# aluo7/ViT-SOM

Measured on AMD Instinct MI355X. Metric: images/sec/node ViT-SOM 40x40 CIFAR-10 bs512 (training step: fwd+bwd+all-reduce+AdamW), higher is better.
Workload: dtype f32 (Linear GEMMs on bf16 MFMA: forward from an exact 3xbf16 operand split, six products; weight / input gradients from a 2xbf16 split, three products, rel. error 4e-6)

## Files before the change

### include/vitsom_hip.h

```cpp
#ifndef VITSOM_HIP_H
#define VITSOM_HIP_H

#include <stddef.h>
#include <stdint.h>

#ifdef __cplusplus
extern "C" {
#endif

typedef struct ihipStream_t* vsom_stream_t;

#define VSOM_OK 0
#define VSOM_EINVAL (-1)
#define VSOM_EALIGN (-2)
#define VSOM_EUNSUPPORTED (-3)
#define VSOM_EWORKSPACE (-4)

#define VSOM_VERSION 100

#define VSOM_DIST_COSINE 0
#define VSOM_DIST_EUCLIDEAN 1
#define VSOM_DIST_MANHATTAN 2

int vsom_version(void);
// ... 39 lines not shown
                         float* dcls_token, int B, int C, int S, int p, int E, void* ws,
                         size_t ws_bytes, vsom_stream_t stream);

int vsom_layernorm_fwd(const float* X, const float* gamma, const float* beta, float* Y, float* mean,
                       float* rstd, int rows, int cols, float eps, vsom_stream_t stream);
size_t vsom_layernorm_bwd_workspace_bytes(int rows, int cols);
int vsom_layernorm_bwd(const float* dY, const float* X, const float* mean, const float* rstd,
                       const float* gamma, const float* resid, float* dX, float* dgamma, float* dbeta,
                       int rows, int cols, void* ws, size_t ws_bytes, vsom_stream_t stream);
#define VSOM_LN_JOB_WORDS 4
int vsom_layernorm_bwd_deferrable(int rows, int cols);
int vsom_layernorm_bwd_partial(const float* dY, const float* X, const float* mean, const float* rstd,
                               const float* gamma, const float* resid, float* dX, int rows, int cols, void* part,
                               size_t part_bytes, vsom_stream_t stream);
int vsom_layernorm_bwd_finish_many(const int64_t* jobs_dev, int first, int count, int max_cols, vsom_stream_t stream);

int vsom_attention_fwd(const float* qkv, float* out, float* lse, int B, int N, int H, int hd,
                       vsom_stream_t stream);
int vsom_attention_bwd(const float* qkv, const float* out, const float* dout, const float* lse,
                       float* dqkv, float* delta_ws, int B, int N, int H, int hd,
                       vsom_stream_t stream);
int vsom_attention_probs(const float* qkv, const float* lse, float* probs, int B, int N, int H, int hd,
                         vsom_stream_t stream);
int vsom_set_attention_fused(int fused);

int vsom_attention_q1_fwd(const float* q, const float* kv, float* o, float* lse, int B, int N, int H, int hd,
                          vsom_stream_t stream);
int vsom_attention_q1_bwd(const float* dout, const float* o, const float* lse, const float* q, const float* kv, float* dq,
                          float* dkv, int B, int N, int H, int hd, vsom_stream_t stream);
int vsom_rows_add(const float* src, long lds, float* dst, long ldd, int rows, int cols, vsom_stream_t stream);
// ... 122 lines not shown
```

### vit_som_amd/_lib.py

```python
import ctypes as C
import os

import torch

_HERE = os.path.dirname(os.path.abspath(__file__))
LIB_PATH = os.path.join(_HERE, "libvitsom_hip.so")

c_fp = C.c_void_p
c_stream = C.c_void_p

SIGNATURES = {
    "vsom_version": (C.c_int, []),
    "vsom_last_error_string": (C.c_char_p, []),
    "vsom_linear_fwd": (C.c_int, [c_fp, C.c_long, c_fp, c_fp, c_fp, C.c_long, C.c_int, C.c_int, C.c_int, c_stream]),
    "vsom_linear_gelu_fwd": (C.c_int, [c_fp, C.c_long, c_fp, c_fp, c_fp, c_fp, C.c_int, C.c_int, C.c_int, c_stream]),
    "vsom_linear_relu_fwd": (C.c_int, [c_fp, C.c_long, c_fp, c_fp, c_fp, c_fp, C.c_int, C.c_int, C.c_int, c_stream]),
    "vsom_l1_loss_workspace_bytes": (C.c_size_t, [C.c_long]),
    "vsom_l1_loss": (C.c_int, [c_fp, c_fp, c_fp, c_fp, C.c_float, C.c_long, c_fp, C.c_size_t, c_stream]),
    "vsom_linear_residual_fwd": (C.c_int, [c_fp, C.c_long, c_fp, c_fp, c_fp, C.c_long, C.c_int, c_fp, C.c_long,
                                           C.c_int, C.c_int, C.c_int, c_stream]),
    "vsom_linear_bwd_input": (C.c_int, [c_fp, C.c_long, c_fp, c_fp, C.c_long, C.c_int, C.c_int, C.c_int, C.c_int,
                                        c_fp, c_stream]),
    "vsom_linear_bwd_input_t": (C.c_int, [c_fp, C.c_long, c_fp, c_fp, C.c_long, C.c_int, C.c_int, C.c_int, C.c_int,
                                          c_fp, c_stream]),
# ... 2 lines not shown
    "vsom_get_gemm_mode": (C.c_int, []),
    "vsom_linear_bwd_weight_workspace_bytes": (C.c_size_t, [C.c_int, C.c_int, C.c_int]),
    "vsom_linear_bwd_weight": (C.c_int, [c_fp, C.c_long, c_fp, C.c_long, c_fp, c_fp, C.c_int, C.c_int, C.c_int,
                                         c_fp, C.c_size_t, c_stream]),
    "vsom_patch_embed_fwd": (C.c_int, [c_fp, c_fp, c_fp, c_fp, c_fp, c_fp, c_fp, C.c_int, C.c_int, C.c_int, C.c_int,
                                       C.c_int, c_stream]),
    "vsom_patch_embed_bwd_workspace_bytes": (C.c_size_t, [C.c_int] * 5),
    "vsom_patch_embed_bwd": (C.c_int, [c_fp, c_fp, c_fp, c_fp, c_fp, C.c_int, C.c_int, C.c_int, C.c_int, C.c_int,
                                       c_fp, C.c_size_t, c_stream]),
    "vsom_layernorm_fwd": (C.c_int, [c_fp, c_fp, c_fp, c_fp, c_fp, c_fp, C.c_int, C.c_int, C.c_float, c_stream]),
    "vsom_layernorm_bwd_workspace_bytes": (C.c_size_t, [C.c_int, C.c_int]),
    "vsom_layernorm_bwd": (C.c_int, [c_fp] * 9 + [C.c_int, C.c_int, c_fp, C.c_size_t, c_stream]),
    "vsom_layernorm_bwd_deferrable": (C.c_int, [C.c_int, C.c_int]),
    "vsom_layernorm_bwd_partial": (C.c_int, [c_fp] * 7 + [C.c_int, C.c_int, c_fp, C.c_size_t, c_stream]),
    "vsom_layernorm_bwd_finish_many": (C.c_int, [c_fp, C.c_int, C.c_int, C.c_int, c_stream]),
    "vsom_attention_fwd": (C.c_int, [c_fp, c_fp, c_fp, C.c_int, C.c_int, C.c_int, C.c_int, c_stream]),
    "vsom_attention_bwd": (C.c_int, [c_fp] * 6 + [C.c_int] * 4 + [c_stream]),
    "vsom_set_attention_fused": (C.c_int, [C.c_int]),
    "vsom_attention_probs": (C.c_int, [c_fp, c_fp, c_fp, C.c_int, C.c_int, C.c_int, C.c_int, c_stream]),
    "vsom_attention_q1_fwd": (C.c_int, [c_fp] * 4 + [C.c_int] * 4 + [c_stream]),
    "vsom_attention_q1_bwd": (C.c_int, [c_fp] * 7 + [C.c_int] * 4 + [c_stream]),
    "vsom_rows_add": (C.c_int, [c_fp, C.c_long, c_fp, C.c_long, C.c_int, C.c_int, c_stream]),
    "vsom_tape_begin": (C.c_int, []),
    "vsom_tape_cut": (C.c_int, []),
    "vsom_tape_pause": (C.c_int, [C.c_int]),
    "vsom_tape_end": (C.c_int, []),
    "vsom_tape_recording": (C.c_int, []),
    "vsom_tape_segment_ops": (C.c_int, [C.c_int, C.c_int]),
    "vsom_tape_replay": (C.c_int, [C.c_int, C.c_int]),
    "vsom_tape_destroy": (C.c_int, [C.c_int]),
# ... 170 lines not shown
```

### vit_som_amd/csrc/gemm_f32.h

```cpp
#pragma once
#include "common.h"

namespace vsom {

enum Epi : int {
    EPI_NONE = 0,
    EPI_BIAS = 1,
    EPI_BIAS_GELU = 2,
    EPI_BIAS_RES = 3,
    EPI_ROWAXPY = 4,
    EPI_GELU_BWD = 5,
    EPI_SLAB = 6,
    EPI_BIAS_RELU = 7,
};

struct GemmP {
    const float* A; const float* B; float* C;
    long lda, ldb, ldc;
    int M, N, K;
    int ktiles_per_split;
    int a_seg, a_stride, a_off;
    int c_seg, c_stride, c_off;
    const float* bias;
    const float* R; long ldr; int r_mod, r_off;
    float* C2; long ldc2;
    const float* rowscale;
    float alpha; int accumulate;
    float* slab; long slab_stride;
    float* slab_bias; long slab_bias_stride;
    int n_major;
    int a_vec, b_vec;
    unsigned a_bytes, b_bytes;
    int products;
};

template <int R_>
struct StageRegs { f32x4 v[R_ / 32]; };

constexpr unsigned OOB = 0xFFFFFFF0u;

__device__ __forceinline__ f32x4 bload4(__amdgpu_buffer_rsrc_t rsrc, unsigned off) {
    return __builtin_bit_cast(f32x4, __builtin_amdgcn_raw_buffer_load_b128(rsrc, (int)off, 0, 0));
}

__device__ __forceinline__ f32x4 bload4s(__amdgpu_buffer_rsrc_t rsrc, unsigned voff, unsigned soff) {
    return __builtin_bit_cast(f32x4, __builtin_amdgcn_raw_buffer_load_b128(rsrc, (int)voff, (int)soff, 0));
}

// ... 445 lines not shown
```

### vit_som_amd/csrc/gemm_f32.hip

```cpp
#include "gemm_f32.h"
#include "gemm_x6.h"
#include "gemm_x6_tn.h"

#include <atomic>

#include <stdarg.h>
#include <stdlib.h>

namespace vsom {

static thread_local char g_err[512] = "no error";
void set_error(const char* fmt, ...) {
    va_list ap;
    va_start(ap, fmt);
    vsnprintf(g_err, sizeof(g_err), fmt, ap);
    va_end(ap);
}
const char* last_error() { return g_err; }

static std::atomic<int> g_gemm_mode{VSOM_GEMM_SPLIT_BF16_GRAD3};
int gemm_mode() { return g_gemm_mode.load(std::memory_order_relaxed); }
static bool split_engine() { return gemm_mode() != VSOM_GEMM_F32; }
int gemm_grad_products() { return gemm_mode() == VSOM_GEMM_SPLIT_BF16_GRAD3 ? 3 : 6; }

// ... 165 lines not shown
    p.cfg = (N % 192 == 0 && K % 64 == 0) ? 1 : (N % 96 == 0 && K % 96 == 0) ? 2 : 0;
    if (p.cfg == 0) {
        p.splits = choose_splits(cdiv(N, gemm_tile_m(false, false, N)) * cdiv(K, 64), cdiv(M, 32), 128);
        return p;
    }
    const int tiles = p.cfg == 1 ? (N / 192) * (K / 64) : (N / 96) * (K / 96);
    const int ktiles = cdiv(M, 32);
    int s = (384 + tiles / 2) / tiles;
    if (s > ktiles) s = ktiles;
    if (s < 1) s = 1;
    const int per = cdiv(ktiles, s);
    p.splits = cdiv(ktiles, per);
    return p;
}
static long pad4(long n) { return (n + 3) & ~3L; }


int linear_bwd_weight_impl(const float* dY, long lddy, const float* X, long ldx, float* dW, float* db, int M, int N,
                           int K, int a_seg, int a_stride, int a_off, void* ws, size_t ws_bytes,
                           hipStream_t stream) {
    VSOM_REQUIRE(dY && X && dW, VSOM_EINVAL, "linear_bwd_weight: null pointer");
    VSOM_REQUIRE(lddy >= N && ldx >= K, VSOM_EINVAL, "linear_bwd_weight: leading dimension too small");
    VSOM_REQUIRE(ws && ws_bytes >= vsom_linear_bwd_weight_workspace_bytes(M, N, K), VSOM_EWORKSPACE,
                 "linear_bwd_weight: workspace too small (%zu < %zu)", ws_bytes,
                 vsom_linear_bwd_weight_workspace_bytes(M, N, K));
    VSOM_REQUIRE(aligned16(ws), VSOM_EALIGN, "linear_bwd_weight: workspace must be 16-byte aligned");
    const TnPlan plan = bwd_weight_plan(M, N, K);
    const int splits = plan.splits;
    const long wlen = pad4((long)N * K), blen = pad4(N);
    float* slab = static_cast<float*>(ws);
// ... 108 lines not shown
int vsom_linear_bwd_input_t(const float* dY, long lddy, const float* Wt, float* dX, long lddx, int M, int N, int K,
                            int accumulate, const float* gelu_grad, vsom_stream_t stream) {
    VSOM_REQUIRE(dY && Wt && dX, VSOM_EINVAL, "linear_bwd_input_t: null pointer");
    VSOM_REQUIRE(lddy >= N && lddx >= K, VSOM_EINVAL, "linear_bwd_input_t: leading dimension too small");
    GemmP g = {};
    g.A = dY; g.lda = lddy; g.B = Wt; g.ldb = N; g.C = dX; g.ldc = lddx;
    g.M = M; g.N = K; g.K = N; g.alpha = 1.f; g.accumulate = accumulate;
    g.products = gemm_grad_products();
    if (gelu_grad) {
        g.R = gelu_grad; g.ldr = K;
        return launch_gemm(true, true, EPI_GELU_BWD, g, 1, stream);
    }
    return launch_gemm(true, true, EPI_NONE, g, 1, stream);
}

int vsom_set_gemm_mode(int mode) {
    VSOM_REQUIRE(mode == VSOM_GEMM_F32 || mode == VSOM_GEMM_SPLIT_BF16 || mode == VSOM_GEMM_SPLIT_BF16_GRAD3, VSOM_EINVAL,
                 "set_gemm_mode: unknown mode %d", mode);
    g_gemm_mode.store(mode, std::memory_order_relaxed);
    return VSOM_OK;
}
int vsom_get_gemm_mode(void) { return gemm_mode(); }

size_t vsom_linear_bwd_weight_workspace_bytes(int M, int N, int K) {
    if (M <= 0 || N <= 0 || K <= 0) return 0;
    const int s = bwd_weight_plan(M, N, K).splits;
    return (size_t)s * (size_t)(pad4((long)N * K) + pad4(N)) * sizeof(float);
}

int vsom_linear_bwd_weight(const float* dY, long lddy, const float* X, long ldx, float* dW, float* db, int M,
// ... 6 lines not shown
```

### vit_som_amd/csrc/gemm_x6.h

```cpp
#pragma once
#include "gemm_f32.h"

namespace vsom {

typedef __attribute__((ext_vector_type(8))) __bf16 bf16x8;

__device__ __forceinline__ unsigned x6_bits(float x) { return __builtin_bit_cast(unsigned, x); }
__device__ __forceinline__ float x6_float(unsigned x) { return __builtin_bit_cast(float, x); }

__device__ __forceinline__ void x6_split(f32x4 v, uint2& p1, uint2& p2, uint2& p3) {
    const unsigned HI = 0xffff0000u, SEL = 0x07060302u;
    float r[4], s[4];
#pragma unroll
    for (int e = 0; e < 4; ++e) {
        r[e] = v[e] - x6_float(x6_bits(v[e]) & HI);
        s[e] = r[e] - x6_float(x6_bits(r[e]) & HI);
    }
    p1.x = __builtin_amdgcn_perm(x6_bits(v[1]), x6_bits(v[0]), SEL); p1.y = __builtin_amdgcn_perm(x6_bits(v[3]), x6_bits(v[2]), SEL);
    p2.x = __builtin_amdgcn_perm(x6_bits(r[1]), x6_bits(r[0]), SEL); p2.y = __builtin_amdgcn_perm(x6_bits(r[3]), x6_bits(r[2]), SEL);
    p3.x = __builtin_amdgcn_perm(x6_bits(s[1]), x6_bits(s[0]), SEL); p3.y = __builtin_amdgcn_perm(x6_bits(s[3]), x6_bits(s[2]), SEL);
}

typedef __attribute__((ext_vector_type(2))) __bf16 bf16x2_t;
__device__ __forceinline__ void x3_split(f32x4 v, uint2& p1, uint2& p2) {
// ... 36 lines not shown
}
template <int NPL = 3>
__device__ __forceinline__ void x6_store_ks(const X6Blk& b, char* planes, int plane_bytes, int mq, int kg) {
#pragma unroll
    for (int e = 0; e < 4; ++e) {
        const f32x4 col = {b.v[0][e], b.v[1][e], b.v[2][e], b.v[3][e]};
        uint2 p1, p2, p3;
        if constexpr (NPL == 3) x6_split(col, p1, p2, p3); else x3_split(col, p1, p2);
        char* dst = planes + x6_piece_off(4 * mq + e, kg);
        *reinterpret_cast<uint2*>(dst) = p1;
        *reinterpret_cast<uint2*>(dst + plane_bytes) = p2;
        if constexpr (NPL == 3) *reinterpret_cast<uint2*>(dst + 2 * plane_bytes) = p3;
    }
}

template <bool A_KC, bool B_KC, int WM, int WN, int WAVES_M, int WAVES_N, int EPI, int NPL = 3>
__global__ __launch_bounds__(256) void gemm_x6_kernel(const GemmP g) {
    constexpr int BM = WAVES_M * WM * 32;
    constexpr int BN = WAVES_N * WN * 32;
    constexpr int PA = BM * X6_RS, PB = BN * X6_RS;
    __shared__ __attribute__((aligned(16))) char lds[NPL * (PA + PB)];
    char* As = lds;
    char* Bs = lds + NPL * PA;

    const int t = threadIdx.x;
    const int lane = t & 63, wave = t >> 6;
    const int r = lane & 31, h = lane >> 5;
    const int wm0 = (wave / WAVES_N) * (WM * 32);
    const int wn0 = (wave % WAVES_N) * (WN * 32);

    const int tiles_n = (g.N + BN - 1) / BN;
    const int tiles_m = (g.M + BM - 1) / BM;
// ... 13 lines not shown

    f32x16 acc[WM][WN];
#pragma unroll
    for (int i = 0; i < WM; ++i)
#pragma unroll
        for (int j = 0; j < WN; ++j)
#pragma unroll
            for (int v = 0; v < 16; ++v) acc[i][j][v] = 0.f;

    const __amdgpu_buffer_rsrc_t rsA = __builtin_amdgcn_make_buffer_rsrc(const_cast<float*>(g.A), 0, (int)g.a_bytes, 0x00020000);
    const __amdgpu_buffer_rsrc_t rsB = __builtin_amdgcn_make_buffer_rsrc(const_cast<float*>(g.B), 0, (int)g.b_bytes, 0x00020000);
    StageRegs<A_KC ? BM : 32> sa;
    StageRegs<B_KC ? BN : 32> sb;
    OffKC<A_KC ? BM : 32> oa; OffKC<B_KC ? BN : 32> ob;
    constexpr int TA = 2 * BM, TB0 = 256 - 2 * BN;
    static_assert(TA <= 256 && TB0 >= 0, "tile too large for the k-strided task map");
    const bool has_a = !A_KC && t < TA, has_b = !B_KC && t >= TB0;
    const int kga = t & 7, mqa = t >> 3, kgb = (t - TB0) & 7, mqb = (t - TB0) >> 3;
    X6Blk ba, bb;
    unsigned cola = OOB, colb = OOB;
    float cs[4] = {0.f, 0.f, 0.f, 0.f};
    const bool want_colsum = (EPI == EPI_SLAB) && !A_KC && g.slab_bias != nullptr && bn0 == 0;
    if constexpr (A_KC) init_kc<BM>(oa, g.lda, bm0, g.M, t);
    else if (has_a && bm0 + 4 * mqa < g.M) cola = (unsigned)(bm0 + 4 * mqa) << 2;
    if constexpr (B_KC) init_kc<BN>(ob, g.ldb, bn0, g.N, t);
    else if (has_b && bn0 + 4 * mqb < g.N) colb = (unsigned)(bn0 + 4 * mqb) << 2;
    auto gload = [&](int kt) {
        if constexpr (A_KC) load_kc_fast<BM>(sa, rsA, oa, kt << 5, g.K, t);
        else if (has_a) x6_load_ks(ba, rsA, cola, (unsigned)g.lda << 2, kt << 5, g.K, kga, g.a_seg, g.a_stride, g.a_off);
        if constexpr (B_KC) load_kc_fast<BN>(sb, rsB, ob, kt << 5, g.K, t);
        else if (has_b) x6_load_ks(bb, rsB, colb, (unsigned)g.ldb << 2, kt << 5, g.K, kgb, 0, 0, 0);
// ... 58 lines not shown
        lstore();
        __syncthreads();
    }
    if (kt_begin < kt_end) mfma_tile();
    if constexpr (EPI == EPI_SLAB && !A_KC) {
        if (want_colsum && has_a) {
#pragma unroll
            for (int e = 0; e < 4; ++e) {
                float v = cs[e];
                v += __shfl_xor(v, 1, 64); v += __shfl_xor(v, 2, 64); v += __shfl_xor(v, 4, 64);
                const int m = bm0 + 4 * mqa + e;
                if (kga == 0 && m < g.M) g.slab_bias[(long)z * g.slab_bias_stride + m] = v;
            }
        }
    }
    gemm_epilogue<WM, WN, EPI>(g, acc, bm0 + wm0, bn0 + wn0, r, h, z);
}

}
```

### vit_som_amd/csrc/layernorm.hip

```cpp
#include "gemm_f32.h"

namespace vsom {

template <int MAXV>
__global__ __launch_bounds__(256) void layernorm_fwd_kernel(const float* __restrict__ X,
                                                            const float* __restrict__ gamma,
                                                            const float* __restrict__ beta,
                                                            float* __restrict__ Y, float* __restrict__ mean,
                                                            float* __restrict__ rstd, int rows, int cols,
                                                            float eps) {
    const int lane = threadIdx.x & 63;
    const int row = blockIdx.x * 4 + (threadIdx.x >> 6);
    if (row >= rows) return;
    const float* x = X + (long)row * cols;
    float v[MAXV];
    float s = 0.f;
#pragma unroll
    for (int j = 0; j < MAXV; ++j) {
        const int c = lane + 64 * j;
        v[j] = (c < cols) ? x[c] : 0.f;
        s += v[j];
    }
    const float mu = wave_sum(s) / (float)cols;
    float q = 0.f;
// ... 64 lines not shown
            }
        }
    }
#pragma unroll
    for (int j = 0; j < MAXV; ++j) {
        const int c = lane + 64 * j;
        if (c < cols) { sh[(wave * 2 + 0) * cols + c] = dg[j]; sh[(wave * 2 + 1) * cols + c] = db[j]; }
    }
    __syncthreads();
    for (int c = threadIdx.x; c < 2 * cols; c += 256) {
        const float s = (sh[c] + sh[2 * cols + c]) + (sh[4 * cols + c] + sh[6 * cols + c]);
        part[(long)blockIdx.x * 2 * cols + c] = s;
    }
}

__device__ __forceinline__ float group16_sum(float v) {
    v += __shfl_xor(v, 8, 64); v += __shfl_xor(v, 4, 64); v += __shfl_xor(v, 2, 64); v += __shfl_xor(v, 1, 64);
    return v;
}

template <int NCH>
__global__ __launch_bounds__(256) void layernorm_fwd_v4_kernel(const float* __restrict__ X, const float* __restrict__ gamma,
                                                               const float* __restrict__ beta, float* __restrict__ Y,
                                                               float* __restrict__ mean, float* __restrict__ rstd, int rows,
                                                               int cols, float eps) {
    const int sub = threadIdx.x & 15;
    const int row = blockIdx.x * 16 + (threadIdx.x >> 4);
    const bool ok = row < rows;
    const f32x4* x = reinterpret_cast<const f32x4*>(X + (long)(ok ? row : 0) * cols);
    const float inv_n = 1.0f / (float)cols;
    f32x4 v[NCH];
    bool cv[NCH];
    float s = 0.f;
#pragma unroll
// ... 35 lines not shown
    const float inv_n = 1.0f / (float)cols;
    f32x4 gam[NCH], dg[NCH], db[NCH];
    bool cv[NCH];
#pragma unroll
    for (int j = 0; j < NCH; ++j) {
        cv[j] = 4 * (sub + 16 * j) < cols;
        gam[j] = cv[j] ? reinterpret_cast<const f32x4*>(gamma)[sub + 16 * j] : f32x4{0.f, 0.f, 0.f, 0.f};
        dg[j] = f32x4{0.f, 0.f, 0.f, 0.f};
        db[j] = f32x4{0.f, 0.f, 0.f, 0.f};
    }
    for (int row0 = blockIdx.x * 16; row0 < rows; row0 += gridDim.x * 16) {
        const int row = row0 + rg;
        const bool ok = row < rows;
        const long base = (long)(ok ? row : 0) * cols;
        const float mu = mean[ok ? row : 0], rs = rstd[ok ? row : 0];
        f32x4 xh[NCH], g[NCH];
        float s1 = 0.f, s2 = 0.f;
#pragma unroll
        for (int j = 0; j < NCH; ++j) {
            f32x4 d = f32x4{0.f, 0.f, 0.f, 0.f}, xv = f32x4{mu, mu, mu, mu};
            if (cv[j]) {
                xv = reinterpret_cast<const f32x4*>(X + base)[sub + 16 * j];
                if (ok) d = reinterpret_cast<const f32x4*>(dY + base)[sub + 16 * j];
            }
#pragma unroll
            for (int e = 0; e < 4; ++e) {
                xh[j][e] = (xv[e] - mu) * rs;
                g[j][e] = d[e] * gam[j][e];
                s1 += g[j][e];
                s2 = fmaf(g[j][e], xh[j][e], s2);
                dg[j][e] = fmaf(d[e], xh[j][e], dg[j][e]);
                db[j][e] += d[e];
            }
        }
        s1 = group16_sum(s1) * inv_n;
        s2 = group16_sum(s2) * inv_n;
        if (ok) {
#pragma unroll
            for (int j = 0; j < NCH; ++j) {
                if (!cv[j]) continue;
                f32x4 o;
#pragma unroll
                for (int e = 0; e < 4; ++e) o[e] = rs * (g[j][e] - s1 - xh[j][e] * s2);
                if (resid) {
                    const f32x4 rr = reinterpret_cast<const f32x4*>(resid + base)[sub + 16 * j];
#pragma unroll
                    for (int e = 0; e < 4; ++e) o[e] += rr[e];
                }
                reinterpret_cast<f32x4*>(dX + base)[sub + 16 * j] = o;
            }
        }
    }
#pragma unroll
    for (int j = 0; j < NCH; ++j) {
        if (!cv[j]) continue;
        reinterpret_cast<f32x4*>(sh + (rg * 2 + 0) * cols)[sub + 16 * j] = dg[j];
        reinterpret_cast<f32x4*>(sh + (rg * 2 + 1) * cols)[sub + 16 * j] = db[j];
    }
    __syncthreads();
    for (int c = threadIdx.x; c < 2 * cols; c += 256) {
        float s = 0.f;
#pragma unroll
        for (int q = 0; q < 16; ++q) s += sh[q * 2 * cols + c];
        part[(long)blockIdx.x * 2 * cols + c] = s;
// ... 114 lines not shown
```

### vit_som_amd/ops.py

```python
from typing import Optional

import torch

from . import _lib as _lib_mod
from ._lib import check, lib, ptr, stream

_scratch = {}
_retired = []

_timers = {}


def enable_timer(name: str):
    _timers[name] = []


def disable_timers():
    _timers.clear()


def timer_ms(name: str):
    ev = _timers.get(name, [])
    if not ev:
        return None
# ... 196 lines not shown
            del self.keys[i:], self.rows_host[i:], self.parts[i:]
            self.table = None
        if i == len(self.keys):
            nbytes = lib.vsom_layernorm_bwd_workspace_bytes(rows, cols)
            part = torch.empty(nbytes, dtype=torch.uint8, device=self.device)
            self.keys.append(key); self.parts.append(part)
            self.rows_host.append([ptr(part), ptr(dgamma), ptr(dbeta), ((nbytes // (8 * cols)) << 32) | cols])
            self.max_cols = max(self.max_cols, cols)
            self.table = None
        part = self.parts[i]
        check(lib.vsom_layernorm_bwd_partial(ptr(dy), ptr(x), ptr(mean), ptr(rstd), ptr(gamma), ptr(resid), ptr(dx), rows, cols,
                                             ptr(part), part.numel(), stream()), "vsom_layernorm_bwd_partial")
        self.n += 1
        return dx

    def flush(self):
        if self.n == self.flushed:
            return
        if self.table is None or self.table.shape[0] < self.n:
            self.table = torch.tensor(self.rows_host, dtype=torch.int64, device=self.device)
        check(lib.vsom_layernorm_bwd_finish_many(ptr(self.table), self.flushed, self.n - self.flushed, self.max_cols, stream()),
              "vsom_layernorm_bwd_finish_many")
        self.flushed = self.n


def layernorm_bwd_deferrable(rows: int, cols: int) -> bool:
    return bool(lib.vsom_layernorm_bwd_deferrable(int(rows), int(cols)))


def attention_fwd(qkv, out, lse, B, N, H, hd):
    assert qkv.is_contiguous() and out.is_contiguous() and lse.is_contiguous()
    _f32(qkv, "qkv")
    check(lib.vsom_attention_fwd(ptr(qkv), ptr(out), ptr(lse), B, N, H, hd, stream()), "vsom_attention_fwd")
    return out


def attention_bwd(qkv, out, dout, lse, dqkv, delta, B, N, H, hd):
    assert all(t.is_contiguous() for t in (qkv, out, dout, lse, dqkv, delta))
    check(lib.vsom_attention_bwd(ptr(qkv), ptr(out), ptr(dout), ptr(lse), ptr(dqkv), ptr(delta), B, N, H, hd, stream()),
          "vsom_attention_bwd")
    return dqkv

# ... 431 lines not shown
```

### vit_som_amd/tuning.py

```python


class _Hooks:
    side_stream = True
    fwd_split = True
    fwd_split_blocks = None
    overlap_allreduce = True
    bucket_blocks = 3
    bmu_planes = True
    adamw_planes = False
    ln_reduce_batched = True
    bmu_overlap = False
    launch_tape = True
    cls_prune = True

    def set(self, **kw):
        for k, v in kw.items():
            if not hasattr(_Hooks, k):
                raise AttributeError(f"unknown hook {k!r}")
            setattr(self, k, v)
        return self

    def signature(self):
        return tuple((k, getattr(self, k)) for k in sorted(vars(_Hooks)) if not k.startswith("_") and not callable(getattr(_Hooks, k)))

    def reset(self):
        for k in list(self.__dict__):
            delattr(self, k)
        return self
# ... 4 lines not shown
```

### vit_som_amd/vit.py

```python
import math
from typing import Dict

import numpy as np
import torch
import torch.nn as nn

from . import ops
from ._base import _Acts
from ._lib import Event, on_stream
from .tuning import hooks


def _sincos_1d(embed_dim: int, pos: np.ndarray) -> np.ndarray:
    omega = np.arange(embed_dim // 2, dtype=np.float64) / (embed_dim / 2.0)
    omega = 1.0 / 10000 ** omega
    out = np.einsum("m,d->md", pos.reshape(-1).astype(np.float64), omega)
    return np.concatenate([np.sin(out), np.cos(out)], axis=1)


def get_2d_sincos_pos_embed(embed_dim: int, grid_size: int, cls_token: bool = False) -> np.ndarray:
    gh = np.arange(grid_size, dtype=np.float32)
    gw = np.arange(grid_size, dtype=np.float32)
    grid = np.stack(np.meshgrid(gw, gh), axis=0).reshape(2, 1, grid_size, grid_size)
    emb = np.concatenate([_sincos_1d(embed_dim // 2, grid[0]), _sincos_1d(embed_dim // 2, grid[1])], axis=1)
# ... 321 lines not shown
            pend.clear()
            return
        while len(pend) > keep:
            pend.pop(0).wait()

    def _side_mark(self):
        if self._side is not None:
            self.__dict__.setdefault("_side_pending", []).append(self._event().record(self._side))

    def _ln_bwd(self, dy, x, mean, rstd, gamma, resid, dx, dgamma, dbeta):
        jobs = self.__dict__.get("_ln_jobs")
        if jobs is not None and ops.layernorm_bwd_deferrable(*x.shape):
            return jobs.bwd(dy, x, mean, rstd, gamma, resid, dx, dgamma, dbeta)
        return ops.layernorm_bwd(dy, x, mean, rstd, gamma, resid, dx, dgamma, dbeta)

    def _block_bwd(self, blk: Block, L: _Acts, x_in, gout, a: _Acts, G, prefix: str, bufs, WT=None, parity: int = 0):
        T, dim, hid = a.T, blk.dim, blk.hidden
        self._side_join(keep=1)
        g1, g0 = bufs
        dh = a.dh2[parity][:T * hid].view(T, hid)
        da = a.da[:T * dim].view(T, dim)
        dqkv = a.dqkv2[parity][:T * 3 * dim].view(T, 3 * dim)
        self._dw(gout, L.hact, G(f"{prefix}.mlp.2.weight"), G(f"{prefix}.mlp.2.bias"))
        self._dx(WT, gout, blk.mlp["2"].weight, dh, gelu_grad=L.hpre)
        self._dw(dh, L.a2, G(f"{prefix}.mlp.0.weight"), G(f"{prefix}.mlp.0.bias"))
        self._dx(WT, dh, blk.mlp["0"].weight, da)
        self._ln_bwd(da, L.x1, L.mean2, L.rstd2, blk.norm2.weight, gout, g1, G(f"{prefix}.norm2.weight"),
                          G(f"{prefix}.norm2.bias"))
        self._dw(g1, L.ao, G(f"{prefix}.attn.proj.weight"), G(f"{prefix}.attn.proj.bias"))
        self._dx(WT, g1, blk.attn.proj.weight, da)
        ops.attention_bwd(L.qkv, L.ao, da, L.lse, dqkv, a.delta, a.B, a.N, blk.heads, dim // blk.heads)
        self._dw(dqkv, L.a1, G(f"{prefix}.attn.qkv.weight"), G(f"{prefix}.attn.qkv.bias"))
        self._dx(WT, dqkv, blk.attn.qkv.weight, da)
        self._ln_bwd(da, x_in, L.mean1, L.rstd1, blk.norm1.weight, g1, g0, G(f"{prefix}.norm1.weight"),
                          G(f"{prefix}.norm1.bias"))
        self._side_mark()
        return g0

    def _views(self, a: _Acts, dim: int):
        return [b[:a.T * dim].view(a.T, dim) for b in a.g]

    def _decoder_bwd(self, a: _Acts, G, WT=None, before_dxe=None):
        DE = self.decoder_embed_dim
        ring = self._views(a, DE)
        gA = ring[0]
        ops.linear_bwd_weight(a.dpred, a.dn, G("decoder_pred.weight"), G("decoder_pred.bias"))
        dn_grad = a.da[:a.T * DE].view(a.T, DE)
        self._dx(WT, a.dpred, self.decoder_pred.weight, dn_grad)
        x_last = a.dec[-1].x2 if a.dec else a.dec0
        self._ln_bwd(dn_grad, x_last, a.mean_d, a.rstd_d, self.decoder_norm.weight, None, gA,
# ... 116 lines not shown
```

Measured before the change: 54180.

## Fuse LayerNorm backward into the input-gradient GEMM epilogue

Adds a GEMM kernel variant whose epilogue computes the LayerNorm backward for full-width row tiles (K=192 or 96). It writes dX with the residual added and emits per-tile dgamma/dbeta partials, which are reduced later or deferred through the existing LN job queue. The transformer block backward now uses this fused path for norm2 and norm1. This removes the intermediate da write/read and one kernel launch per LayerNorm. In exchange, whole-row tiles may reduce GEMM parallelism and raise register pressure.

```diff
diff --git a/include/vitsom_hip.h b/include/vitsom_hip.h
--- a/include/vitsom_hip.h
+++ b/include/vitsom_hip.h
@@ -77,6 +77,15 @@
                                const float* gamma, const float* resid, float* dX, int rows, int cols, void* part,
                                size_t part_bytes, vsom_stream_t stream);
 int vsom_layernorm_bwd_finish_many(const int64_t* jobs_dev, int first, int count, int max_cols, vsom_stream_t stream);
+
+int vsom_linear_bwd_input_ln_supported(int M, int N, int K);
+size_t vsom_linear_bwd_input_ln_partial_bytes(int M, int K);
+int vsom_linear_bwd_input_ln(const float* dY, long lddy, const float* Wt, int M, int N, int K, const float* X,
+                             const float* mean, const float* rstd, const float* gamma, const float* resid, float* dX,
+                             float* dgamma, float* dbeta, void* ws, size_t ws_bytes, vsom_stream_t stream);
+int vsom_linear_bwd_input_ln_partial(const float* dY, long lddy, const float* Wt, int M, int N, int K, const float* X,
+                                     const float* mean, const float* rstd, const float* gamma, const float* resid,
+                                     float* dX, void* part, size_t part_bytes, vsom_stream_t stream);
 
 int vsom_attention_fwd(const float* qkv, float* out, float* lse, int B, int N, int H, int hd,
                        vsom_stream_t stream);
diff --git a/vit_som_amd/_lib.py b/vit_som_amd/_lib.py
--- a/vit_som_amd/_lib.py
+++ b/vit_som_amd/_lib.py
@@ -40,6 +40,10 @@
     "vsom_layernorm_bwd_deferrable": (C.c_int, [C.c_int, C.c_int]),
     "vsom_layernorm_bwd_partial": (C.c_int, [c_fp] * 7 + [C.c_int, C.c_int, c_fp, C.c_size_t, c_stream]),
     "vsom_layernorm_bwd_finish_many": (C.c_int, [c_fp, C.c_int, C.c_int, C.c_int, c_stream]),
+    "vsom_linear_bwd_input_ln_supported": (C.c_int, [C.c_int, C.c_int, C.c_int]),
+    "vsom_linear_bwd_input_ln_partial_bytes": (C.c_size_t, [C.c_int, C.c_int]),
+    "vsom_linear_bwd_input_ln": (C.c_int, [c_fp, C.c_long, c_fp, C.c_int, C.c_int, C.c_int] + [c_fp] * 8 + [c_fp, C.c_size_t, c_stream]),
+    "vsom_linear_bwd_input_ln_partial": (C.c_int, [c_fp, C.c_long, c_fp, C.c_int, C.c_int, C.c_int] + [c_fp] * 6 + [c_fp, C.c_size_t, c_stream]),
     "vsom_attention_fwd": (C.c_int, [c_fp, c_fp, c_fp, C.c_int, C.c_int, C.c_int, C.c_int, c_stream]),
     "vsom_attention_bwd": (C.c_int, [c_fp] * 6 + [C.c_int] * 4 + [c_stream]),
     "vsom_set_attention_fused": (C.c_int, [C.c_int]),
diff --git a/vit_som_amd/csrc/gemm_f32.h b/vit_som_amd/csrc/gemm_f32.h
--- a/vit_som_amd/csrc/gemm_f32.h
+++ b/vit_som_amd/csrc/gemm_f32.h
@@ -12,6 +12,7 @@
     EPI_GELU_BWD = 5,
     EPI_SLAB = 6,
     EPI_BIAS_RELU = 7,
+    EPI_LN_BWD = 8,
 };
 
 struct GemmP {
@@ -32,6 +33,8 @@
     int a_vec, b_vec;
     unsigned a_bytes, b_bytes;
     int products;
+    const float* ln_x; const float* ln_mean; const float* ln_rstd; const float* ln_gamma; const float* ln_resid;
+    float* ln_part;
 };
 
 template <int R_>
diff --git a/vit_som_amd/csrc/gemm_f32.hip b/vit_som_amd/csrc/gemm_f32.hip
--- a/vit_som_amd/csrc/gemm_f32.hip
+++ b/vit_som_amd/csrc/gemm_f32.hip
@@ -203,6 +203,43 @@
     return p;
 }
 static long pad4(long n) { return (n + 3) & ~3L; }
+
+static bool ln_fused_width(int K) { return K == 192 || K == 96; }
+static int ln_fused_tiles(int M, int K) { return cdiv(M, K == 192 ? 64 : 128); }
+
+static int linear_bwd_input_ln_launch(const float* dY, long lddy, const float* Wt, int M, int N, int K, const float* X,
+                                      const float* mean, const float* rstd, const float* gamma, const float* resid,
+                                      float* dX, float* part, size_t part_bytes, hipStream_t stream) {
+    VSOM_REQUIRE(dY && Wt && X && mean && rstd && gamma && dX, VSOM_EINVAL, "linear_bwd_input_ln: null pointer");
+    VSOM_REQUIRE(M > 0 && N > 0 && lddy >= N, VSOM_EINVAL, "linear_bwd_input_ln: bad shape M=%d N=%d lddy=%ld", M, N, lddy);
+    VSOM_REQUIRE(vsom_linear_bwd_input_ln_supported(M, N, K), VSOM_EUNSUPPORTED,
+                 "linear_bwd_input_ln: unsupported (M=%d N=%d K=%d, gemm mode %d)", M, N, K, gemm_mode());
+    VSOM_REQUIRE(aligned16(dY) && aligned16(Wt) && aligned16(X) && aligned16(gamma) && aligned16(dX) &&
+                 (!resid || aligned16(resid)) && lddy % 4 == 0 && N % 4 == 0, VSOM_EALIGN,
+                 "linear_bwd_input_ln: operands must be 16-byte aligned (lddy, N multiples of 4)");
+    VSOM_REQUIRE(part && aligned16(part) && part_bytes >= vsom_linear_bwd_input_ln_partial_bytes(M, K), VSOM_EWORKSPACE,
+                 "linear_bwd_input_ln: partial buffer too small or misaligned");
+    const long ab = operand_bytes(M, lddy, N), bb = operand_bytes(K, N, N);
+    VSOM_REQUIRE(ab < 0xFFFF0000L && (long)M * K * 4 < 0xFFFF0000L, VSOM_EUNSUPPORTED, "linear_bwd_input_ln: operand larger than 4 GB");
+    GemmP g = {};
+    g.A = dY; g.lda = lddy; g.B = Wt; g.ldb = N; g.C = dX; g.ldc = K;
+    g.M = M; g.N = K; g.K = N; g.alpha = 1.f;
+    g.ktiles_per_split = cdiv(N, 32);
+    g.a_vec = g.b_vec = 1;
+    g.a_bytes = (unsigned)ab; g.b_bytes = (unsigned)bb;
+    g.products = gemm_grad_products();
+    g.ln_x = X; g.ln_mean = mean; g.ln_rstd = rstd; g.ln_gamma = gamma; g.ln_resid = resid; g.ln_part = part;
+    const dim3 grid(ln_fused_tiles(M, K)), block(256);
+    const bool x3 = g.products == 3;
+    if (K == 192) {
+        if (x3) VSOM_LAUNCH((gemm_x6_ln_kernel<3, 2, 2, 2>), grid, block, 0, stream, g);
+        else VSOM_LAUNCH((gemm_x6_ln_kernel<3, 2, 2, 3>), grid, block, 0, stream, g);
+    } else {
+        if (x3) VSOM_LAUNCH((gemm_x6_ln_kernel<3, 4, 1, 2>), grid, block, 0, stream, g);
+        else VSOM_LAUNCH((gemm_x6_ln_kernel<3, 4, 1, 3>), grid, block, 0, stream, g);
+    }
+    VSOM_LAUNCH_CHECK("gemm_x6_ln_kernel");
+}
 
 
 int linear_bwd_weight_impl(const float* dY, long lddy, const float* X, long ldx, float* dW, float* db, int M, int N,
@@ -341,6 +378,32 @@
     return launch_gemm(true, true, EPI_NONE, g, 1, stream);
 }
 
+int vsom_linear_bwd_input_ln_supported(int M, int N, int K) {
+    return M > 0 && N > 0 && split_engine() && ln_fused_width(K) && ln_fused_tiles(M, K) >= 32;
+}
+
+size_t vsom_linear_bwd_input_ln_partial_bytes(int M, int K) {
+    if (M <= 0 || !ln_fused_width(K)) return 0;
+    return (size_t)ln_fused_tiles(M, K) * 2 * (size_t)K * sizeof(float);
+}
+
+int vsom_linear_bwd_input_ln(const float* dY, long lddy, const float* Wt, int M, int N, int K, const float* X,
+                             const float* mean, const float* rstd, const float* gamma, const float* resid, float* dX,
+                             float* dgamma, float* dbeta, void* ws, size_t ws_bytes, vsom_stream_t stream) {
+    VSOM_REQUIRE(dgamma && dbeta, VSOM_EINVAL, "linear_bwd_input_ln: null pointer");
+    float* part = static_cast<float*>(ws);
+    const int rc = linear_bwd_input_ln_launch(dY, lddy, Wt, M, N, K, X, mean, rstd, gamma, resid, dX, part, ws_bytes, stream);
+    if (rc) return rc;
+    return reduce_slabs2_internal(part, 2L * K, ln_fused_tiles(M, K), dgamma, K, dbeta, K, K, stream);
+}
+
+int vsom_linear_bwd_input_ln_partial(const float* dY, long lddy, const float* Wt, int M, int N, int K, const float* X,
+                                     const float* mean, const float* rstd, const float* gamma, const float* resid,
+                                     float* dX, void* part, size_t part_bytes, vsom_stream_t stream) {
+    return linear_bwd_input_ln_launch(dY, lddy, Wt, M, N, K, X, mean, rstd, gamma, resid, dX, static_cast<float*>(part),
+                                      part_bytes, stream);
+}
+
 int vsom_set_gemm_mode(int mode) {
     VSOM_REQUIRE(mode == VSOM_GEMM_F32 || mode == VSOM_GEMM_SPLIT_BF16 || mode == VSOM_GEMM_SPLIT_BF16_GRAD3, VSOM_EINVAL,
                  "set_gemm_mode: unknown mode %d", mode);
diff --git a/vit_som_amd/csrc/gemm_x6.h b/vit_som_amd/csrc/gemm_x6.h
--- a/vit_som_amd/csrc/gemm_x6.h
+++ b/vit_som_amd/csrc/gemm_x6.h
@@ -1,9 +1,11 @@
 #pragma once
 #include "gemm_f32.h"
+#include "layernorm_bwd.h"
 
 namespace vsom {
 
 typedef __attribute__((ext_vector_type(8))) __bf16 bf16x8;
+typedef unsigned v4u32 __attribute__((ext_vector_type(4)));
 
 __device__ __forceinline__ unsigned x6_bits(float x) { return __builtin_bit_cast(unsigned, x); }
 __device__ __forceinline__ float x6_float(unsigned x) { return __builtin_bit_cast(float, x); }
@@ -74,8 +76,101 @@
     }
 }
 
+template <int WN, int WAVES_M, int WAVES_N, int LDS_BYTES>
+__device__ __forceinline__ void x6_ln_bwd_epilogue(const GemmP& g, const f32x16 (&acc)[1][WN], char* lds, int bm0, int wm0,
+                                                   int wn0, int r, int h, int tile) {
+    constexpr int BN = WAVES_N * WN * 32;
+    constexpr int cols = BN;
+    constexpr int NCH = (BN + 63) / 64;
+    constexpr int LROW = BN + 8;
+    constexpr int PROWS = WAVES_M * 8;
+    constexpr int ITER = PROWS / 16;
+    static_assert(PROWS % 16 == 0 && PROWS * LROW * 4 <= LDS_BYTES && 16 * 2 * BN * 4 <= LDS_BYTES, "LN epilogue does not fit");
+    float* st = reinterpret_cast<float*>(lds);
+    const int t = threadIdx.x, sub = t & 15, rg = t >> 4;
+    const float inv_n = 1.0f / (float)cols;
+    const unsigned rbytes = (unsigned)g.M * cols * 4u;
+    const __amdgpu_buffer_rsrc_t rsX = __builtin_amdgcn_make_buffer_rsrc(const_cast<float*>(g.ln_x), 0, (int)rbytes, 0x00020000);
+    const __amdgpu_buffer_rsrc_t rsR = __builtin_amdgcn_make_buffer_rsrc(const_cast<float*>(g.ln_resid), 0, (int)rbytes, 0x00020000);
+    const __amdgpu_buffer_rsrc_t rsD = __builtin_amdgcn_make_buffer_rsrc(g.C, 0, (int)rbytes, 0x00020000);
+    const __amdgpu_buffer_rsrc_t rsM = __builtin_amdgcn_make_buffer_rsrc(const_cast<float*>(g.ln_mean), 0, g.M * 4, 0x00020000);
+    const __amdgpu_buffer_rsrc_t rsS = __builtin_amdgcn_make_buffer_rsrc(const_cast<float*>(g.ln_rstd), 0, g.M * 4, 0x00020000);
+    const bool has_resid = g.ln_resid != nullptr;
+    f32x4 gam[NCH], dg[NCH], db[NCH];
+    bool cv[NCH];
+#pragma unroll
+    for (int j = 0; j < NCH; ++j) {
+        cv[j] = 4 * (sub + 16 * j) < cols;
+        gam[j] = cv[j] ? reinterpret_cast<const f32x4*>(g.ln_gamma)[sub + 16 * j] : f32x4{0.f, 0.f, 0.f, 0.f};
+        dg[j] = f32x4{0.f, 0.f, 0.f, 0.f};
+        db[j] = f32x4{0.f, 0.f, 0.f, 0.f};
+    }
+    const int wr = wm0 >> 5;
+#pragma unroll
+    for (int q = 0; q < 4; ++q) {
+        bool ok[ITER];
+        unsigned off[ITER][NCH];
+        float mu[ITER], rs[ITER];
+        f32x4 xv[ITER][NCH], rr[ITER][NCH];
+#pragma unroll
+        for (int i = 0; i < ITER; ++i) {
+            const int lr = 16 * i + rg;
+            const int row = bm0 + (lr >> 3) * 32 + 8 * q + (lr & 7);
+            ok[i] = row < g.M;
+#pragma unroll
+            for (int j = 0; j < NCH; ++j)
+                off[i][j] = (ok[i] && cv[j]) ? (unsigned)row * (cols * 4u) + 16u * (sub + 16 * j) : OOB;
+            const unsigned roff = ok[i] ? (unsigned)row * 4u : OOB;
+            mu[i] = __builtin_bit_cast(float, __builtin_amdgcn_raw_buffer_load_b32(rsM, (int)roff, 0, 0));
+            rs[i] = __builtin_bit_cast(float, __builtin_amdgcn_raw_buffer_load_b32(rsS, (int)roff, 0, 0));
+#pragma unroll
+            for (int j = 0; j < NCH; ++j) {
+                xv[i][j] = bload4(rsX, off[i][j]);
+                rr[i][j] = has_resid ? bload4(rsR, off[i][j]) : f32x4{0.f, 0.f, 0.f, 0.f};
+            }
+        }
+        __syncthreads();
+#pragma unroll
+        for (int j = 0; j < WN; ++j)
+#pragma unroll
+            for (int e = 0; e < 4; ++e) st[(wr * 8 + e + 4 * h) * LROW + wn0 + j * 32 + r] = acc[0][j][4 * q + e];
+        __syncthreads();
+#pragma unroll
+        for (int i = 0; i < ITER; ++i) {
+            const int lr = 16 * i + rg;
+            f32x4 d[NCH], o[NCH];
+#pragma unroll
+            for (int j = 0; j < NCH; ++j) {
+                d[j] = (cv[j] && ok[i]) ? *reinterpret_cast<const f32x4*>(st + lr * LROW + 4 * (sub + 16 * j)) : f32x4{0.f, 0.f, 0.f, 0.f};
+                if (!cv[j]) xv[i][j] = f32x4{mu[i], mu[i], mu[i], mu[i]};
+            }
+            ln_bwd_row<NCH>(d, xv[i], mu[i], rs[i], gam, inv_n, o, dg, db);
+#pragma unroll
+            for (int j = 0; j < NCH; ++j) {
+                if (has_resid) ln_bwd_add_resid(o[j], rr[i][j]);
+                __builtin_amdgcn_raw_buffer_store_b128(__builtin_bit_cast(v4u32, o[j]), rsD, (int)off[i][j], 0, 0);
+            }
+        }
+    }
+    __syncthreads();
+    float* sh = st;
+#pragma unroll
+    for (int j = 0; j < NCH; ++j) {
+        if (!cv[j]) continue;
+        reinterpret_cast<f32x4*>(sh + (rg * 2 + 0) * cols)[sub + 16 * j] = dg[j];
+        reinterpret_cast<f32x4*>(sh + (rg * 2 + 1) * cols)[sub + 16 * j] = db[j];
+    }
+    __syncthreads();
+    for (int c = t; c < 2 * cols; c += 256) {
+        float s = 0.f;
+#pragma unroll
+        for (int q = 0; q < 16; ++q) s += sh[q * 2 * cols + c];
+        g.ln_part[(long)tile * 2 * cols + c] = s;
+    }
+}
+
 template <bool A_KC, bool B_KC, int WM, int WN, int WAVES_M, int WAVES_N, int EPI, int NPL = 3>
-__global__ __launch_bounds__(256) void gemm_x6_kernel(const GemmP g) {
+__device__ __forceinline__ void gemm_x6_body(const GemmP& g) {
     constexpr int BM = WAVES_M * WM * 32;
     constexpr int BN = WAVES_N * WN * 32;
     constexpr int PA = BM * X6_RS, PB = BN * X6_RS;
@@ -119,7 +214,7 @@
     StageRegs<B_KC ? BN : 32> sb;
     OffKC<A_KC ? BM : 32> oa; OffKC<B_KC ? BN : 32> ob;
     constexpr int TA = 2 * BM, TB0 = 256 - 2 * BN;
-    static_assert(TA <= 256 && TB0 >= 0, "tile too large for the k-strided task map");
+    static_assert((A_KC || TA <= 256) && (B_KC || TB0 >= 0), "tile too large for the k-strided task map");
     const bool has_a = !A_KC && t < TA, has_b = !B_KC && t >= TB0;
     const int kga = t & 7, mqa = t >> 3, kgb = (t - TB0) & 7, mqb = (t - TB0) >> 3;
     X6Blk ba, bb;
@@ -208,7 +303,22 @@
             }
         }
     }
-    gemm_epilogue<WM, WN, EPI>(g, acc, bm0 + wm0, bn0 + wn0, r, h, z);
-}
-
-}
+    if constexpr (EPI == EPI_LN_BWD) {
+        static_assert(A_KC && B_KC && WM == 1, "EPI_LN_BWD: NT GEMM, one accumulator row per wave");
+        x6_ln_bwd_epilogue<WN, WAVES_M, WAVES_N, (int)sizeof(lds)>(g, acc, lds, bm0, wm0, wn0, r, h, tm);
+    } else {
+        gemm_epilogue<WM, WN, EPI>(g, acc, bm0 + wm0, bn0 + wn0, r, h, z);
+    }
+}
+
+template <bool A_KC, bool B_KC, int WM, int WN, int WAVES_M, int WAVES_N, int EPI, int NPL = 3>
+__global__ __launch_bounds__(256) void gemm_x6_kernel(const GemmP g) {
+    gemm_x6_body<A_KC, B_KC, WM, WN, WAVES_M, WAVES_N, EPI, NPL>(g);
+}
+
+template <int WN, int WAVES_M, int WAVES_N, int NPL>
+__global__ __launch_bounds__(256, 2) void gemm_x6_ln_kernel(const GemmP g) {
+    gemm_x6_body<true, true, 1, WN, WAVES_M, WAVES_N, EPI_LN_BWD, NPL>(g);
+}
+
+}
diff --git a/vit_som_amd/csrc/layernorm.hip b/vit_som_amd/csrc/layernorm.hip
--- a/vit_som_amd/csrc/layernorm.hip
+++ b/vit_som_amd/csrc/layernorm.hip
@@ -1,4 +1,5 @@
 #include "gemm_f32.h"
+#include "layernorm_bwd.h"
 
 namespace vsom {
 
@@ -102,10 +103,6 @@
     }
 }
 
-__device__ __forceinline__ float group16_sum(float v) {
-    v += __shfl_xor(v, 8, 64); v += __shfl_xor(v, 4, 64); v += __shfl_xor(v, 2, 64); v += __shfl_xor(v, 1, 64);
-    return v;
-}
 
 template <int NCH>
 __global__ __launch_bounds__(256) void layernorm_fwd_v4_kernel(const float* __restrict__ X, const float* __restrict__ gamma,
@@ -171,40 +168,25 @@
         const bool ok = row < rows;
         const long base = (long)(ok ? row : 0) * cols;
         const float mu = mean[ok ? row : 0], rs = rstd[ok ? row : 0];
-        f32x4 xh[NCH], g[NCH];
-        float s1 = 0.f, s2 = 0.f;
+        f32x4 d[NCH], xv[NCH], o[NCH];
 #pragma unroll
         for (int j = 0; j < NCH; ++j) {
-            f32x4 d = f32x4{0.f, 0.f, 0.f, 0.f}, xv = f32x4{mu, mu, mu, mu};
+            d[j] = f32x4{0.f, 0.f, 0.f, 0.f};
+            xv[j] = f32x4{mu, mu, mu, mu};
             if (cv[j]) {
-                xv = reinterpret_cast<const f32x4*>(X + base)[sub + 16 * j];
-                if (ok) d = reinterpret_cast<const f32x4*>(dY + base)[sub + 16 * j];
+                xv[j] = reinterpret_cast<const f32x4*>(X + base)[sub + 16 * j];
+                if (ok) d[j] = reinterpret_cast<const f32x4*>(dY + base)[sub + 16 * j];
             }
-#pragma unroll
-            for (int e = 0; e < 4; ++e) {
-                xh[j][e] = (xv[e] - mu) * rs;
-                g[j][e] = d[e] * gam[j][e];
-                s1 += g[j][e];
-                s2 = fmaf(g[j][e], xh[j][e], s2);
-                dg[j][e] = fmaf(d[e], xh[j][e], dg[j][e]);
-                db[j][e] += d[e];
-            }
-        }
-        s1 = group16_sum(s1) * inv_n;
-        s2 = group16_sum(s2) * inv_n;
+        }
+        ln_bwd_row<NCH>(d, xv, mu, rs, gam, inv_n, o, dg, db);
         if (ok) {
 #pragma unroll
             for (int j = 0; j < NCH; ++j) {
                 if (!cv[j]) continue;
-                f32x4 o;
-#pragma unroll
-                for (int e = 0; e < 4; ++e) o[e] = rs * (g[j][e] - s1 - xh[j][e] * s2);
                 if (resid) {
-                    const f32x4 rr = reinterpret_cast<const f32x4*>(resid + base)[sub + 16 * j];
-#pragma unroll
-                    for (int e = 0; e < 4; ++e) o[e] += rr[e];
+                    ln_bwd_add_resid(o[j], reinterpret_cast<const f32x4*>(resid + base)[sub + 16 * j]);
                 }
-                reinterpret_cast<f32x4*>(dX + base)[sub + 16 * j] = o;
+                reinterpret_cast<f32x4*>(dX + base)[sub + 16 * j] = o[j];
             }
         }
     }
diff --git a/vit_som_amd/csrc/layernorm_bwd.h b/vit_som_amd/csrc/layernorm_bwd.h
--- /dev/null
+++ b/vit_som_amd/csrc/layernorm_bwd.h
@@ -0,0 +1,44 @@
+#pragma once
+#include "common.h"
+
+namespace vsom {
+
+__device__ __forceinline__ float group16_sum(float v) {
+    v += __shfl_xor(v, 8, 64); v += __shfl_xor(v, 4, 64); v += __shfl_xor(v, 2, 64); v += __shfl_xor(v, 1, 64);
+    return v;
+}
+
+template <int NCH>
+__device__ __forceinline__ void ln_bwd_row(const f32x4 (&d)[NCH], const f32x4 (&xv)[NCH], float mu, float rs,
+                                           const f32x4 (&gam)[NCH], float inv_n, f32x4 (&o)[NCH], f32x4 (&dg)[NCH],
+                                           f32x4 (&db)[NCH]) {
+#pragma clang fp contract(off)
+    f32x4 xh[NCH], g[NCH];
+    float s1 = 0.f, s2 = 0.f;
+#pragma unroll
+    for (int j = 0; j < NCH; ++j) {
+#pragma unroll
+        for (int e = 0; e < 4; ++e) {
+            xh[j][e] = (xv[j][e] - mu) * rs;
+            g[j][e] = d[j][e] * gam[j][e];
+            s1 += g[j][e];
+            s2 = fmaf(g[j][e], xh[j][e], s2);
+            dg[j][e] = fmaf(d[j][e], xh[j][e], dg[j][e]);
+            db[j][e] += d[j][e];
+        }
+    }
+    s1 = group16_sum(s1) * inv_n;
+    s2 = group16_sum(s2) * inv_n;
+#pragma unroll
+    for (int j = 0; j < NCH; ++j)
+#pragma unroll
+        for (int e = 0; e < 4; ++e) o[j][e] = rs * fmaf(-xh[j][e], s2, g[j][e] - s1);
+}
+
+__device__ __forceinline__ void ln_bwd_add_resid(f32x4& o, const f32x4& rr) {
+#pragma clang fp contract(off)
+#pragma unroll
+    for (int e = 0; e < 4; ++e) o[e] += rr[e];
+}
+
+}
diff --git a/vit_som_amd/ops.py b/vit_som_amd/ops.py
--- a/vit_som_amd/ops.py
+++ b/vit_som_amd/ops.py
@@ -234,6 +234,25 @@
         self.n += 1
         return dx
 
+    def bwd_linear_fused(self, dy, Wt, x, mean, rstd, gamma, resid, dx, dgamma, dbeta):
+        rows, cols = x.shape
+        key = (ptr(dgamma), ptr(dbeta), rows, cols, "fused")
+        i = self.n
+        if i < len(self.keys) and self.keys[i] != key:
+            del self.keys[i:], self.rows_host[i:], self.parts[i:]
+            self.table = None
+        if i == len(self.keys):
+            nbytes = lib.vsom_linear_bwd_input_ln_partial_bytes(rows, cols)
+            part = torch.empty(nbytes, dtype=torch.uint8, device=self.device)
+            self.keys.append(key); self.parts.append(part)
+            self.rows_host.append([ptr(part), ptr(dgamma), ptr(dbeta), ((nbytes // (8 * cols)) << 32) | cols])
+            self.max_cols = max(self.max_cols, cols)
+            self.table = None
+        part = self.parts[i]
+        linear_bwd_input_ln_partial(dy, Wt, x, mean, rstd, gamma, resid, dx, part)
+        self.n += 1
+        return dx
+
     def flush(self):
         if self.n == self.flushed:
             return
@@ -246,6 +265,33 @@
 
 def layernorm_bwd_deferrable(rows: int, cols: int) -> bool:
     return bool(lib.vsom_layernorm_bwd_deferrable(int(rows), int(cols)))
+
+
+def linear_bwd_input_ln_supported(rows: int, n: int, cols: int) -> bool:
+    return bool(lib.vsom_linear_bwd_input_ln_supported(int(rows), int(n), int(cols)))
+
+
+def _ln_fused_args(dy, Wt, x, mean, rstd, gamma, resid, dx):
+    M, N = dy.shape
+    K = Wt.shape[0]
+    for n_, t in (("dy", dy), ("Wt", Wt), ("x", x), ("dx", dx)):
+        _f32(t, n_)
+    assert Wt.shape[1] == N and Wt.is_contiguous() and x.shape == (M, K) == dx.shape and x.is_contiguous() and dx.is_contiguous()
+    assert resid is None or (resid.is_contiguous() and resid.shape == (M, K))
+    return (ptr(dy), _rows(dy), ptr(Wt), M, N, K, ptr(x), ptr(mean), ptr(rstd), ptr(gamma), ptr(resid), ptr(dx))
+
+
+def linear_bwd_input_ln(dy, Wt, x, mean, rstd, gamma, resid, dx, dgamma, dbeta):
+    args = _ln_fused_args(dy, Wt, x, mean, rstd, gamma, resid, dx)
+    ws = scratch(lib.vsom_linear_bwd_input_ln_partial_bytes(x.shape[0], x.shape[1]), x.device)
+    check(lib.vsom_linear_bwd_input_ln(*args, ptr(dgamma), ptr(dbeta), ptr(ws), ws.numel(), stream()), "vsom_linear_bwd_input_ln")
+    return dx
+
+
+def linear_bwd_input_ln_partial(dy, Wt, x, mean, rstd, gamma, resid, dx, part):
+    args = _ln_fused_args(dy, Wt, x, mean, rstd, gamma, resid, dx)
+    check(lib.vsom_linear_bwd_input_ln_partial(*args, ptr(part), part.numel(), stream()), "vsom_linear_bwd_input_ln_partial")
+    return dx
 
 
 def attention_fwd(qkv, out, lse, B, N, H, hd):
diff --git a/vit_som_amd/tuning.py b/vit_som_amd/tuning.py
--- a/vit_som_amd/tuning.py
+++ b/vit_som_amd/tuning.py
@@ -12,6 +12,7 @@
     bmu_overlap = False
     launch_tape = True
     cls_prune = True
+    ln_bwd_fused = True
 
     def set(self, **kw):
         for k, v in kw.items():
diff --git a/vit_som_amd/vit.py b/vit_som_amd/vit.py
--- a/vit_som_amd/vit.py
+++ b/vit_som_amd/vit.py
@@ -359,6 +359,16 @@
             return jobs.bwd(dy, x, mean, rstd, gamma, resid, dx, dgamma, dbeta)
         return ops.layernorm_bwd(dy, x, mean, rstd, gamma, resid, dx, dgamma, dbeta)
 
+    def _dx_ln(self, WT, dy, weight, da, x, mean, rstd, gamma, resid, dx, dgamma, dbeta):
+        wt = WT(weight) if (WT is not None and hooks.ln_bwd_fused) else None
+        if wt is not None and ops.linear_bwd_input_ln_supported(dy.shape[0], dy.shape[1], x.shape[1]):
+            jobs = self.__dict__.get("_ln_jobs")
+            if jobs is not None:
+                return jobs.bwd_linear_fused(dy, wt, x, mean, rstd, gamma, resid, dx, dgamma, dbeta)
+            return ops.linear_bwd_input_ln(dy, wt, x, mean, rstd, gamma, resid, dx, dgamma, dbeta)
+        self._dx(WT, dy, weight, da)
+        return self._ln_bwd(da, x, mean, rstd, gamma, resid, dx, dgamma, dbeta)
+
     def _block_bwd(self, blk: Block, L: _Acts, x_in, gout, a: _Acts, G, prefix: str, bufs, WT=None, parity: int = 0):
         T, dim, hid = a.T, blk.dim, blk.hidden
         self._side_join(keep=1)
@@ -369,16 +379,14 @@
         self._dw(gout, L.hact, G(f"{prefix}.mlp.2.weight"), G(f"{prefix}.mlp.2.bias"))
         self._dx(WT, gout, blk.mlp["2"].weight, dh, gelu_grad=L.hpre)
         self._dw(dh, L.a2, G(f"{prefix}.mlp.0.weight"), G(f"{prefix}.mlp.0.bias"))
-        self._dx(WT, dh, blk.mlp["0"].weight, da)
-        self._ln_bwd(da, L.x1, L.mean2, L.rstd2, blk.norm2.weight, gout, g1, G(f"{prefix}.norm2.weight"),
-                          G(f"{prefix}.norm2.bias"))
+        self._dx_ln(WT, dh, blk.mlp["0"].weight, da, L.x1, L.mean2, L.rstd2, blk.norm2.weight, gout, g1,
+                    G(f"{prefix}.norm2.weight"), G(f"{prefix}.norm2.bias"))
         self._dw(g1, L.ao, G(f"{prefix}.attn.proj.weight"), G(f"{prefix}.attn.proj.bias"))
         self._dx(WT, g1, blk.attn.proj.weight, da)
         ops.attention_bwd(L.qkv, L.ao, da, L.lse, dqkv, a.delta, a.B, a.N, blk.heads, dim // blk.heads)
         self._dw(dqkv, L.a1, G(f"{prefix}.attn.qkv.weight"), G(f"{prefix}.attn.qkv.bias"))
-        self._dx(WT, dqkv, blk.attn.qkv.weight, da)
-        self._ln_bwd(da, x_in, L.mean1, L.rstd1, blk.norm1.weight, g1, g0, G(f"{prefix}.norm1.weight"),
-                          G(f"{prefix}.norm1.bias"))
+        self._dx_ln(WT, dqkv, blk.attn.qkv.weight, da, x_in, L.mean1, L.rstd1, blk.norm1.weight, g1, g0,
+                    G(f"{prefix}.norm1.weight"), G(f"{prefix}.norm1.bias"))
         self._side_mark()
         return g0
 
```

Result: faster. 55380 (median of 6 runs) (+2.2%).
